# kentril0/WaterSurfaceRendering

Hardware: AMD Instinct MI355X
Metric: ocean frames/s (ComputeWaves, 7 fields -> displacement + normal map) (higher is better)
Workload: dtype f32; 1 GPU; 2048x2048 tile, FULL7, reference default parameters; tile_size=2048, tiles_per_rank=1, pipeline_depth=3, seed=1592590336, parallelism=tiles sharded 1 process per GPU x1, no data-path collective

## Files before the change

watersurfacerendering_amd/csrc/ocean_kernels.h:

```cpp
#pragma once
#include <hip/hip_runtime.h>
#include <hip/hip_fp16.h>
#include <stdint.h>
#include <type_traits>
#include "fft_engine.h"

namespace ocean {

typedef float ocean_f4 __attribute__((ext_vector_type(4)));
__device__ __forceinline__ void store_nt(float4* p, float4 v)
{
    ocean_f4 t = {v.x, v.y, v.z, v.w};
    __builtin_nontemporal_store(t, reinterpret_cast<ocean_f4*>(p));
}
__device__ __forceinline__ void store_f2_sc1(float2* base, unsigned byte_off, float2 v)
{
    typedef float f2v __attribute__((ext_vector_type(2)));
    const f2v t = {v.x, v.y};
    asm volatile("global_store_dwordx2 %0, %1, %2 sc1" ::"v"(byte_off), "v"(t), "s"(base) : "memory");
}
template <bool NTS> __device__ __forceinline__ void store_map(float4* base, unsigned texel, float4 v)
{
    float4* p = reinterpret_cast<float4*>(reinterpret_cast<char*>(base) + (texel * 16u));
    if constexpr (NTS) store_nt(p, v);
// ... 660 lines not shown

template <int N> constexpr size_t zpass_c1_lds_bytes() { return sizeof(c32) * fft_lds_elems<N, 1>() + sizeof(float) * N; }
template <int N, int T, bool FAST> constexpr int zpass_c1_min_waves() { return T == N / 16 ? 3 : (FAST ? 6 : 5); }
template <int N, int T, class P, bool ZNT = false, bool Z16 = false, bool FAST = true, bool ZWT = false>
__global__ void __launch_bounds__(T, (zpass_c1_min_waves<N, T, FAST>())) k_zpass_c1(const FrameArgs a)
{
    extern __shared__ __attribute__((aligned(16))) unsigned char smem[];
    c32* fbuf = reinterpret_cast<c32*>(smem);
    float* sp = reinterpret_cast<float*>(fbuf + fft_lds_elems<N, 1>());
    float* raw = reinterpret_cast<float*>(fbuf);
    const int tid = threadIdx.x;
    const int tile = blockIdx.y;
#ifdef OCEAN_CLOCKPROBE
    ClockProbe clock_probe_(a.frame_seq);
#endif
    start_ramp_wait(a.start_ramp, blockIdx.x, gridDim.x);
    TwiddleRegs<N, 1, T, P> twr;
    twr.load(a.tw, tid);
#ifdef OCEAN_DEVELOPER
    const int bxr = (blockIdx.x % 8 == 0 || a.xcd_rot == 0) ? (int)blockIdx.x : (int)(blockIdx.x / 8 * 8 + 1 + (blockIdx.x % 8 - 1 + a.xcd_rot) % 7);
    const int nb = xcd_swizzle(bxr, N / 2 + 1);
#else
    const int nb = xcd_swizzle((int)blockIdx.x, N / 2 + 1);
#endif
    const float t = a.t + (a.toff ? a.toff[tile] : 0.0f);
    const float* __restrict__ k1 = a.k1d + (size_t)tile * N;
    const bool col0 = (nb == 0);
    const float h16s = a.h0h ? a.h0_inv_scale[tile] : 1.0f;
    const float base = a.omega_q ? a.base_freq[tile] : 0.0f;
    spectrum_form<FAST>(a, [&](auto h16, auto w16) {
        constexpr bool H16 = decltype(h16)::value, W16 = decltype(w16)::value;
        constexpr int PAIRS = N / 2;
        constexpr int P1 = (PAIRS + T - 1) / T;
        constexpr int PB = P1 > 4 ? 4 : P1;
        static_assert(P1 % PB == 0 && PAIRS % T == 0, "phase-1 batches");
#pragma unroll 1
        for (int ub = 0; ub < P1; ub += PB) {
            float4 ha[PB];
            float2 hb0[PB], hb1[PB], wv[PB];
#pragma unroll
            for (int u = 0; u < PB; ++u)
                zpass_load_pair<N, H16, W16, ZNT>(a, tile, nb, 2 * (tid + (ub + u) * T), h16s, base, ha[u], hb0[u], hb1[u], wv[u]);
#pragma unroll
            for (int u = 0; u < PB; ++u) {
                const int n = 2 * (tid + (ub + u) * T);
                float a0, b0, a1, b1;
                animate_with_mirror(make_float2(ha[u].x, ha[u].y), hb0[u], wv[u].x, t, a0, b0);
                animate_with_mirror(make_float2(ha[u].z, ha[u].w), hb1[u], wv[u].y, t, a1, b1);
                *reinterpret_cast<float2*>(sp + n) = col0 ? make_float2(a0, a1) : make_float2(0.5f * (a0 + b0), 0.5f * (a1 + b1));
                if (n == 0) raw[0] = 0.5f * (a0 - b0);
            }
        }
    });
    if (blockIdx.x == 0 && tid == 0 && (a.zmask & 8)) {
        a.minmax[2 * tile + 0] = float_key(3.402823466e+38f);
        a.minmax[2 * tile + 1] = float_key(1.175494351e-38f);
        a.hdone[tile] = 0u;
    }
    float kzr[P::r[0]];
#pragma unroll
    for (int i = 0; i < P::r[0]; ++i) kzr[i] = k1[tid + i * (N / P::r[0])];
    __syncthreads();
    const float sm0 = raw[0];
    static_assert(!ZWT || (!ZNT && !Z16), "write-through is a policy of the plain fp32 intermediates");
    if (col0) zpass_single_transforms<N, T, P, true, ZNT, Z16, ZWT>(a, fbuf, sp, kzr, twr, k1[nb], sm0, tid, tile, nb);
    else zpass_single_transforms<N, T, P, false, ZNT, Z16, ZWT>(a, fbuf, sp, kzr, twr, k1[nb], sm0, tid, tile, nb);
#ifdef OCEAN_CLOCKPROBE
    clock_probe_.end();
#endif
}
template <int N> constexpr bool zpass_has_c1() { return N >= 1024; }
template <int N> inline bool zpass_c1_pays(bool nt_inter, unsigned tiles)
{
    if (N == 4096) return true;
    if (nt_inter) return false;
    return N == 2048 || tiles >= 2;
}

template <int N, int T> constexpr int zpass_blocks_per_cu()
{
    constexpr int by_lds = (int)(163840 / (sizeof(c32) * fft_lds_elems<N, zpass_columns<N>()>() + sizeof(float) * 2 * N));
    constexpr int by_threads = 2048 / T;
    constexpr int by_regs = (zpass_min_waves<N>() * 4 * 64) / T;
    constexpr int m = by_lds < by_threads ? by_lds : by_threads;
    return (by_regs >= 1 && by_regs < m) ? by_regs : (m < 1 ? 1 : m);
}

template <int N, int ZW = 1> constexpr size_t zpass_lds_bytes()
{
    return sizeof(c32) * fft_lds_elems<N, zpass_columns<N>()>() + sizeof(float) * 2 * N;
}


__device__ __forceinline__ void store_wt(float* p, float v) { __hip_atomic_store(p, v, __ATOMIC_RELAXED, __HIP_MEMORY_SCOPE_AGENT); }
__device__ __forceinline__ float load_wt(const float* p) { return __hip_atomic_load(p, __ATOMIC_RELAXED, __HIP_MEMORY_SCOPE_AGENT); }
__device__ __forceinline__ unsigned load_wt(const unsigned* p) { return __hip_atomic_load(p, __ATOMIC_RELAXED, __HIP_MEMORY_SCOPE_AGENT); }
__device__ __forceinline__ void wait_counter(const unsigned* ctr, unsigned target, int tid, int poll_sleep = 0, unsigned* fault = nullptr)
{
    if (tid == 0) {
#ifdef OCEAN_FAULT_INJECT
        target += 1u;
#endif
        const unsigned long long t0 = wall_clock64();
        bool ok;
        while (!(ok = load_wt(ctr) >= target) && (wall_clock64() - t0) < 2000000ull) {
            if (poll_sleep <= 0) __builtin_amdgcn_s_sleep(2);
            else for (int k = 0; k < poll_sleep; ++k) __builtin_amdgcn_s_sleep(127);
        }
        if (!ok && fault) *fault = 1u;
    }
    __syncthreads();
}

__device__ __forceinline__ void wait_counter_reached(const unsigned* ctr, unsigned target, int tid, int poll_sleep = 0, unsigned* fault = nullptr)
{
    if (tid == 0) {
        const unsigned long long t0 = wall_clock64();
        bool ok;
        while (!(ok = (int)(load_wt(ctr) - target) >= 0) && (wall_clock64() - t0) < 2000000ull) {
            if (poll_sleep <= 0) __builtin_amdgcn_s_sleep(2);
            else for (int k = 0; k < poll_sleep; ++k) __builtin_amdgcn_s_sleep(127);
        }
        if (!ok && fault) *fault = 1u;
    }
    __syncthreads();
}

template <int N, bool Z16 = false>
__device__ __forceinline__ c32 load_pair_column(const float2* __restrict__ zg, int mf, int u, float eps, float unscale = 1.0f, float unscale_y = 0.0f)
{
    using HF = Half<N>;
    if (mf <= N / 2) return load_z<Z16>(zg, HF::template zidx<Z16>(mf, 0, u), unscale, unscale_y);
    const int side = (u == 0 || u == N / 2) ? 0 : 1;
    if constexpr (Z16) return load_z<true>(zg, HF::template zidx<Z16>(N - mf, side, u), eps * unscale, eps * unscale_y);
    const c32 v = load_z<false>(zg, HF::template zidx<Z16>(N - mf, side, u), 1.0f);
    return make_float2(eps * v.x, eps * v.y);
}

template <class LS, int T, class F>
__device__ __forceinline__ void for_each_output(int tid, F f)
{
#pragma unroll
    for (int u = 0; u < LS::IT; ++u) {
        const int w = tid + u * T;
        if (!LS::GUARD || w < LS::ITEMS) {
            int c, j;
            LS::map(w, c, j);
#pragma unroll
            for (int i = 0; i < LS::RL; ++i) f(j + i * LS::STRIDE, c, u, i);
        }
    }
}

template <int N, int C> constexpr bool xpass_single_row_group() { return C > 1 && N >= 1024 && (N / 2) % (2 * C) == 0; }
template <int N, int C> constexpr int xpass_height_groups() { return (N / 2 + 1 + 2 * C - 1) / (2 * C); }

constexpr unsigned DONE_GROUPS = 1024, DONE_STRIDE = 16;
template <int T>
__device__ __forceinline__ void frame_done(const FrameArgs& a, unsigned* lds_flag, int tid, unsigned total = 0, unsigned id = 0)
{
    asm volatile("s_waitcnt vmcnt(0)" ::: "memory");
    __syncthreads();
    if (tid == 0) {
        if (total == 0) { total = gridDim.x * gridDim.y; id = blockIdx.y * gridDim.x + blockIdx.x; }
        const unsigned groups = total / 16u < DONE_GROUPS ? (total + 15u) / 16u : DONE_GROUPS;
        const unsigned g = id % groups, members = total / groups + (g < total % groups ? 1u : 0u);
        unsigned* gc = a.done_ctr + (1u + g) * DONE_STRIDE;
        bool last = false;
        if (atomicAdd(gc, 1u) == members - 1u) {
            *gc = 0u;
            last = atomicAdd(a.done_ctr, 1u) == groups - 1u;
        }
        lds_flag[0] = last;
    }
    __syncthreads();
    if (!lds_flag[0]) return;
    if (tid == 0) *a.done_ctr = 0u;
    for (unsigned i = (unsigned)tid; i < gridDim.y; i += (unsigned)T)
        a.done_rec[i] = make_uint4(load_wt(a.minmax + 2 * i + 0), load_wt(a.minmax + 2 * i + 1), a.frame_seq, 0u);
}


template <int T>
__device__ __forceinline__ void frame_records(const FrameArgs& a, unsigned* lds_flag, int tid, bool first_of_tile, unsigned total = 0, unsigned id = 0)
{
    if (a.rec_mode == 1) {
        if (first_of_tile && tid == 0) a.done_rec[blockIdx.y] = make_uint4(load_wt(a.minmax + 2 * blockIdx.y + 0), load_wt(a.minmax + 2 * blockIdx.y + 1), a.frame_seq, 0u);
    } else if (a.rec_mode == 2) {
        frame_done<T>(a, lds_flag, tid, total, id);
    }
}

template <int N, int C, int T, class P, bool NTS, bool Z16, bool JAC, bool ONE = false>
__device__ __forceinline__ void xpass_b_body(const FrameArgs& a, unsigned char* smem, const int bx, const unsigned rec_total = 0, const unsigned rec_id = 0)
{
    using HF = Half<N>;
    c32* fbuf = reinterpret_cast<c32*>(smem);
    const int tid = threadIdx.x;
    const int tile = blockIdx.y;
    constexpr int LM = 1;
    TwiddleRegs<N, C, T, P, LM> twr;
    twr.load(a.tw, tid);
    constexpr int NB = (HF::NU + C - 1) / C;
    constexpr int HB = JAC ? NB : xpass_height_groups<N, C>();
    static_assert(HF::NUP % (2 * C) == 0, "height row blocks");
    if constexpr (ONE) wait_counter_reached(a.zdone + tile, a.zdone_target, tid, a.poll_sleep, a.fault);

    auto pair3_role = [&]() {
    if constexpr (JAC) {
        {
            constexpr int NW = (T + 63) / 64;
            float* red = reinterpret_cast<float*>(fbuf + fft_lds_elems<N, C>());
            const int u0 = xcd_swizzle(bx, HB) * C;
            const float2* __restrict__ z3 = reinterpret_cast<const float2*>(reinterpret_cast<const char*>(a.z3) + (size_t)tile * HF::Z_GROUP * (Z16 ? 4 : 8));
            float* __restrict__ hraw = a.hraw + (size_t)tile * HF::HRAW_TILE;
            float* __restrict__ jraw = a.jraw + (size_t)tile * HF::HRAW_TILE;
            [[maybe_unused]] float ux = 1.0f, uy = 1.0f;
            float ig = 1.0f;
            { const float4 zs3 = a.zscale[2 * tile + 1]; ig = zs3.w; if constexpr (Z16) { ux = zs3.z; uy = zs3.z; } }
            float vmin = 3.402823466e+38f, vmax = -3.402823466e+38f;
            auto in = [&](int nf, int c, int, int) -> c32 { return load_pair_column<N, Z16>(z3, nf, u0 + c, 1.0f, ux, uy); };
            auto out = [&](int p, int c, c32 v, int, int) {
                const int q = u0 + c;
                if (q > N / 2) return;
                const float s = ((p + q) & 1) ? -1.0f : 1.0f;
                const float ha = s * v.x;
                vmin = fminf(vmin, ha); vmax = fmaxf(vmax, ha);
                at32(hraw, hraw_index(N, p, q)) = ha;
                at32(jraw, hraw_index(N, p, q)) = s * v.y * ig;
            };
            batch_fft<N, C, T, P>(fbuf, twr, tid, in, out);
#pragma unroll
            for (int o = 32; o > 0; o >>= 1) {
                vmin = fminf(vmin, __shfl_xor(vmin, o));
                vmax = fmaxf(vmax, __shfl_xor(vmax, o));
            }
            if ((tid & 63) == 0) { red[tid >> 6] = vmin; red[NW + (tid >> 6)] = vmax; }
            __syncthreads();
            if (tid == 0) {
                for (int w = 1; w < NW; ++w) { vmin = fminf(vmin, red[w]); vmax = fmaxf(vmax, red[NW + w]); }
                atomicMin(a.minmax + 2 * tile + 0, float_key(vmin));
                atomicMax(a.minmax + 2 * tile + 1, float_key(vmax));
            }
        }
    }
    };
    auto height_role = [&]() {
        const bool merged = a.xb_disp != 0;
        constexpr int NW = (T + 63) / 64;
        float* red = reinterpret_cast<float*>(fbuf + fft_lds_elems<N, C>());
        const int u0 = xcd_swizzle(bx, HB) * 2 * C;
        constexpr size_t ES = Z16 ? 4 : 8;
        const float2* __restrict__ zh = reinterpret_cast<const float2*>(reinterpret_cast<const char*>(a.zh) + (size_t)tile * HF::ZH_TILE * ES);
        float* __restrict__ hraw = a.hraw + (size_t)tile * HF::HRAW_TILE;
        float vmin = 3.402823466e+38f, vmax = -3.402823466e+38f;
        [[maybe_unused]] const float uu = Z16 ? a.zscale[2 * tile].z : 1.0f;
        auto in = [&](int nf, int c, int, int) -> c32 {
            const int row = nf <= N / 2 ? nf : N - nf;
            float4 z;
            if constexpr (Z16) {
                const float2 raw2 = *reinterpret_cast<const float2*>(reinterpret_cast<const char*>(zh) + HF::template zhidx<Z16>(row, u0 + 2 * c) * 4u);
                __half2 ha, hb;
                __builtin_memcpy(&ha, &raw2.x, 4); __builtin_memcpy(&hb, &raw2.y, 4);
                const float2 fa = __half22float2(ha), fb = __half22float2(hb);
                z = make_float4(fa.x * uu, fa.y * uu, fb.x * uu, fb.y * uu);
            } else {
                z = *reinterpret_cast<const float4*>(&at32(zh, HF::template zhidx<Z16>(row, u0 + 2 * c)));
            }
            if (nf == 0 || nf == N / 2) return make_float2(z.x, z.z);
            if (nf < N / 2) return make_float2(z.x - z.w, z.y + z.z);
            return make_float2(z.x + z.w, z.z - z.y);
        };
        auto out = [&](int p, int c, c32 v, int, int) {
            const int u = u0 + 2 * c;
            const float s = ((p + u) & 1) ? -1.0f : 1.0f;
            const float ha = s * v.x, hb = -s * v.y;
            if (u <= N / 2) { vmin = fminf(vmin, ha); vmax = fmaxf(vmax, ha); }
            if (u + 1 <= N / 2) { vmin = fminf(vmin, hb); vmax = fmaxf(vmax, hb); }
            if (merged) {
                store_wt(&at32(hraw, hraw_index(N, p, u)), ha);
                store_wt(&at32(hraw, hraw_index(N, p, u + 1)), hb);
            } else {
                at32(hraw, hraw_index(N, p, u)) = ha;
                at32(hraw, hraw_index(N, p, u + 1)) = hb;
            }
        };
        if constexpr (xpass_single_row_group<N, C>()) {
            if (u0 == N / 2) {
                TwiddleRegs<N, 1, T, P, LM> tw1;
                tw1.load(a.tw, tid);
                batch_fft<N, 1, T, P>(fbuf, tw1, tid, in, out);
            } else {
                batch_fft<N, C, T, P>(fbuf, twr, tid, in, out);
            }
        } else {
            batch_fft<N, C, T, P>(fbuf, twr, tid, in, out);
        }
#pragma unroll
        for (int o = 32; o > 0; o >>= 1) {
            vmin = fminf(vmin, __shfl_xor(vmin, o));
            vmax = fmaxf(vmax, __shfl_xor(vmax, o));
        }
        if ((tid & 63) == 0) { red[tid >> 6] = vmin; red[NW + (tid >> 6)] = vmax; }
        __syncthreads();
        if (tid == 0) {
            for (int w = 1; w < NW; ++w) { vmin = fminf(vmin, red[w]); vmax = fmaxf(vmax, red[NW + w]); }
            atomicMin(a.minmax + 2 * tile + 0, float_key(vmin));
            atomicMax(a.minmax + 2 * tile + 1, float_key(vmax));
        }
        if (merged) {
            asm volatile("s_waitcnt vmcnt(0)" ::: "memory");
            __syncthreads();
            if (tid == 0) __hip_atomic_fetch_add(a.hdone + tile, 1u, __ATOMIC_RELAXED, __HIP_MEMORY_SCOPE_AGENT);
        }
    };

    using LS = LastStage<N, C, T, P, LM>;
    auto normal_role = [&]() {
    const int nid = bx - HB;
    const int u0 = (N >= 2048 ? (nid == 0 ? NB - 1 : xcd_swizzle(nid - 1, NB - 1)) : xcd_swizzle(nid, NB)) * C;
    start_ramp_wait(a.start_ramp, (unsigned)nid, (unsigned)NB);
    constexpr size_t ESN = Z16 ? 4 : 8;
    const float2* __restrict__ z1 = reinterpret_cast<const float2*>(reinterpret_cast<const char*>(a.z) + ((size_t)tile * HF::Z_TILE + HF::Z_GROUP) * ESN);
    const float2* __restrict__ z2 = reinterpret_cast<const float2*>(reinterpret_cast<const char*>(z1) + HF::Z_GROUP * ESN);
    [[maybe_unused]] const float uk = Z16 ? a.zscale[2 * tile].w : 1.0f;
    float4* __restrict__ nrm = a.nrm + (size_t)tile * N * N;
    float4* __restrict__ nrm_host = a.nrm_host ? a.nrm_host + (size_t)tile * N * N : nullptr;
    [[maybe_unused]] float* __restrict__ jac0 = JAC ? a.jac0 + (size_t)tile * HF::HRAW_TILE : nullptr;
    [[maybe_unused]] const float lambda = a.lambda ? a.lambda[tile] : a.lambda_all;
    c32 held[LS::IT][LS::RL];
    auto emit = [&](int p, int c, c32 slopes, c32 derivs) {
#pragma clang fp contract(off)
        const int q = u0 + c;
        if (q > N / 2) return;
        const float s = ((p + q) & 1) ? -1.0f : 1.0f;
        const float4 o = make_float4(s * slopes.x, s * slopes.y, s * derivs.x, s * derivs.y);
        if constexpr (JAC)
            at32(jac0, hraw_index(N, p, q)) = (1.0f + lambda * o.z) * (1.0f + lambda * o.w);
        OCEAN_STORE(nrm, q * N + p, o);
        store_map_host(nrm_host, (unsigned)(q * N + p), o);
        if (q != 0 && q != N / 2) {
            OCEAN_STORE(nrm, (N - q) * N + ((N - p) & (N - 1)), make_float4(-o.x, -o.y, o.z, o.w));
            store_map_host(nrm_host, (unsigned)((N - q) * N + ((N - p) & (N - 1))), make_float4(-o.x, -o.y, o.z, o.w));
        }
    };
    const c32 zero = make_float2(0.0f, 0.0f);
    if constexpr (xpass_single_row_group<N, C>()) {
        if (u0 == N / 2) {
            using LS1 = LastStage<N, 1, T, P, LM>;
            if (a.mode == 2) {
                for_each_output<LS1, T>(tid, [&](int p, int c, int, int) { emit(p, c, zero, zero); });
                return;
            }
            TwiddleRegs<N, 1, T, P, LM> tw1;
            tw1.load(a.tw, tid);
            c32 held1[LS1::IT][LS1::RL];
            {
                auto in = [&](int nf, int c, int, int) -> c32 { return load_pair_column<N, Z16>(z1, nf, u0 + c, -1.0f, uk); };
                auto out = [&](int, int, c32 v, int u, int i) { held1[u][i] = v; };
                batch_fft<N, 1, T, P>(fbuf, tw1, tid, in, out);
            }
            if (a.mode == 1) {
                for_each_output<LS1, T>(tid, [&](int p, int c, int u, int i) { emit(p, c, held1[u][i], zero); });
                return;
            }
            __builtin_amdgcn_sched_barrier(0);
            auto in = [&](int nf, int c, int, int) -> c32 { return load_pair_column<N, Z16>(z2, nf, u0 + c, 1.0f, uk); };
            auto out = [&](int p, int c, c32 v, int u, int i) { emit(p, c, held1[u][i], v); };
            batch_fft<N, 1, T, P>(fbuf, tw1, tid, in, out);
            return;
        }
    }
    if (a.mode == 2) {
        for_each_output<LS, T>(tid, [&](int p, int c, int, int) { emit(p, c, zero, zero); });
        return;
    }
    constexpr bool PREFETCH = N >= 2048;
    using FS = FirstStage<N, C, T, P>;
    [[maybe_unused]] c32 xb[PREFETCH ? FS::IT : 1][PREFETCH ? FS::R0 : 1];
    auto fetch = [&](const float2* __restrict__ zg, float eps, auto& dst) {
#pragma unroll
        for (int u = 0; u < FS::IT; ++u) {
            const int w = tid + u * T;
            if (!FS::GUARD || w < FS::ITEMS) {
                const int c = w % C, j = w / C;
#pragma unroll
                for (int i = 0; i < FS::R0; ++i) dst[u][i] = load_pair_column<N, Z16>(zg, j + i * FS::STRIDE, u0 + c, eps, uk);
            }
        }
    };
    if constexpr (PREFETCH) {
        c32 xa[FS::IT][FS::R0];
        fetch(z1, -1.0f, xa);
        if (a.mode != 1) fetch(z2, 1.0f, xb);
        auto in = [&](int, int, int u, int i) -> c32 { return xa[u][i]; };
        auto out = [&](int, int, c32 v, int u, int i) { held[u][i] = v; };
        batch_fft<N, C, T, P>(fbuf, twr, tid, in, out);
    } else {
        auto in = [&](int nf, int c, int, int) -> c32 { return load_pair_column<N, Z16>(z1, nf, u0 + c, -1.0f, uk); };
        auto out = [&](int, int, c32 v, int u, int i) { held[u][i] = v; };
        batch_fft<N, C, T, P>(fbuf, twr, tid, in, out);
    }
    if (a.mode == 1) {
        for_each_output<LS, T>(tid, [&](int p, int c, int u, int i) { emit(p, c, held[u][i], zero); });
        return;
    }
    if constexpr (PREFETCH) {
        auto in = [&](int, int, int u, int i) -> c32 { return xb[u][i]; };
        auto out = [&](int p, int c, c32 v, int u, int i) { emit(p, c, held[u][i], v); };
        batch_fft<N, C, T, P>(fbuf, twr, tid, in, out);
    } else {
        __builtin_amdgcn_sched_barrier(0);
        auto in = [&](int nf, int c, int, int) -> c32 { return load_pair_column<N, Z16>(z2, nf, u0 + c, 1.0f, uk); };
        auto out = [&](int p, int c, c32 v, int u, int i) { emit(p, c, held[u][i], v); };
        batch_fft<N, C, T, P>(fbuf, twr, tid, in, out);
    }
    };
    auto disp_role = [&]() {
        if constexpr (!JAC) {
            using LSD = LastStage<N, C, T, P, LM>;
            const int u0 = xcd_swizzle(bx - HB - NB, NB) * C;
            const float2* __restrict__ z0 = reinterpret_cast<const float2*>(reinterpret_cast<const char*>(a.z) + (size_t)tile * HF::Z_TILE * (Z16 ? 4 : 8));
            [[maybe_unused]] const float uu = Z16 ? a.zscale[2 * tile].z : 1.0f;
            const float* __restrict__ hraw = a.hraw + (size_t)tile * HF::HRAW_TILE;
            float4* __restrict__ disp = a.disp + (size_t)tile * N * N;
            float4* __restrict__ disp_host = a.disp_host ? a.disp_host + (size_t)tile * N * N : nullptr;
            c32 dheld[LSD::IT][LSD::RL];
            if (a.mode != 2) {
                auto in = [&](int nf, int c, int, int) -> c32 { return load_pair_column<N, Z16>(z0, nf, u0 + c, -1.0f, uu); };
                auto out = [&](int, int, c32 v, int u, int i) { dheld[u][i] = v; };
                batch_fft<N, C, T, P>(fbuf, twr, tid, in, out);
            } else {
#pragma unroll
                for (int u = 0; u < LSD::IT; ++u)
#pragma unroll
                    for (int i = 0; i < LSD::RL; ++i) dheld[u][i] = make_float2(0.0f, 0.0f);
            }
            wait_counter(a.hdone + tile, (unsigned)HB, tid, a.poll_sleep, a.fault);
            const unsigned kmn = load_wt(a.minmax + 2 * tile + 0), kmx = load_wt(a.minmax + 2 * tile + 1);
            const float mn = key_float(kmn), mx = key_float(kmx);
            const float inv_a = 1.0f / fmaxf(fabsf(mn), fabsf(mx));
            const float lambda = a.lambda ? a.lambda[tile] : a.lambda_all;
            for_each_output<LSD, T>(tid, [&](int p, int c, int u, int i) {
#pragma clang fp contract(off)
                const int q = u0 + c;
                if (q > N / 2) return;
                const float hv = load_wt(&at32(hraw, hraw_index(N, p, q)));
                const float sg = ((p + q) & 1) ? -1.0f : 1.0f;
                const c32 v = dheld[u][i];
                const float4 o = make_float4(sg * lambda * v.x, hv * inv_a, sg * lambda * v.y, 1.0f);
                store_map<NTS>(disp, (unsigned)(q * N + p), o);
                store_map_host(disp_host, (unsigned)(q * N + p), o);
                if (q != 0 && q != N / 2) {
                    store_map<NTS>(disp, (unsigned)((N - q) * N + ((N - p) & (N - 1))), make_float4(-o.x, o.y, -o.z, 1.0f));
                    store_map_host(disp_host, (unsigned)((N - q) * N + ((N - p) & (N - 1))), make_float4(-o.x, o.y, -o.z, 1.0f));
                }
            });
        }
    };
    const bool merged_launch = a.xb_disp != 0;
    if (bx < HB) { if constexpr (JAC) pair3_role(); else height_role(); }
    else if (!JAC && merged_launch && bx >= HB + NB) disp_role();
    else normal_role();
    frame_records<T>(a, reinterpret_cast<unsigned*>(smem), tid, merged_launch ? bx == HB + NB : bx == HB, rec_total, rec_id);
}

template <int N, int C, int T, class P = Plan<N>, bool NTS = false, bool Z16 = false, bool JAC = false>
__global__ void __launch_bounds__(T) k_xpass_b(const FrameArgs a)
{
    extern __shared__ __attribute__((aligned(16))) unsigned char smem[];
    xpass_b_body<N, C, T, P, NTS, Z16, JAC>(a, smem, (int)blockIdx.x);
}

template <int N, int C, int T, class PZ, class PX, bool NTS, bool Z16, bool FAST>
__global__ void __launch_bounds__(T) k_frame(const FrameArgs a)
{
    extern __shared__ __attribute__((aligned(16))) unsigned char smem[];
    using HF = Half<N>;
    constexpr int NZ = N / 2 + 1;
    constexpr int NB = (HF::NU + C - 1) / C, HB = xpass_height_groups<N, C>();
    const int bx = (int)blockIdx.x;
    if (bx < NZ) {
        zpass_body<N, T, PZ, false, Z16, 1, FAST, true>(a, smem, bx, NZ);
        asm volatile("s_waitcnt vmcnt(0)" ::: "memory");
        __syncthreads();
        if (threadIdx.x == 0) __hip_atomic_fetch_add(a.zdone + blockIdx.y, 1u, __ATOMIC_RELAXED, __HIP_MEMORY_SCOPE_AGENT);
        return;
    }
    xpass_b_body<N, C, T, PX, NTS, Z16, false, true>(a, smem, bx - NZ, (unsigned)(HB + 2 * NB) * gridDim.y, (unsigned)blockIdx.y * (unsigned)(HB + 2 * NB) + (unsigned)(bx - NZ));
}

template <int N, int C, int T, class P = Plan<N>, bool NTS = false, bool Z16 = false, bool JAC = false>
__global__ void __launch_bounds__(T, (T == 512 ? 4 : 1)) k_xpass_disp(const FrameArgs a)
{
    extern __shared__ __attribute__((aligned(16))) unsigned char smem[];
    using HF = Half<N>;
    constexpr int LM = 1;
    c32* fbuf = reinterpret_cast<c32*>(smem);
    const int tid = threadIdx.x;
    const int tile = blockIdx.y;
    constexpr int NB = (HF::NU + C - 1) / C;
    const int u0 = xcd_swizzle(blockIdx.x, NB) * C;
    start_ramp_wait(a.start_ramp, blockIdx.x, gridDim.x);
    const float2* __restrict__ z0 = reinterpret_cast<const float2*>(reinterpret_cast<const char*>(a.z) + (size_t)tile * HF::Z_TILE * (Z16 ? 4 : 8));
    [[maybe_unused]] const float uu = Z16 ? a.zscale[2 * tile].z : 1.0f;
    const float* __restrict__ hraw = a.hraw + (size_t)tile * HF::HRAW_TILE;
    float4* __restrict__ disp = a.disp + (size_t)tile * N * N;
    float4* __restrict__ disp_host = a.disp_host ? a.disp_host + (size_t)tile * N * N : nullptr;
    auto rows = [&](auto cc_tag) {
        constexpr int CC = decltype(cc_tag)::value;
        using LS = LastStage<N, CC, T, P, LM>;
        TwiddleRegs<N, CC, T, P, LM> twr;
        twr.load(a.tw, tid);
        float hv[LS::IT][LS::RL];
        [[maybe_unused]] float jv[JAC ? LS::IT : 1][JAC ? LS::RL : 1], j0[JAC ? LS::IT : 1][JAC ? LS::RL : 1];
#pragma unroll
        for (int u = 0; u < LS::IT; ++u) {
            const int w = tid + u * T;
            if (!LS::GUARD || w < LS::ITEMS) {
                int c, j;
                LS::map(w, c, j);
#pragma unroll
                for (int i = 0; i < LS::RL; ++i) {
                    hv[u][i] = at32(hraw, hraw_index(N, j + i * LS::STRIDE, u0 + c));
                    if constexpr (JAC) {
                        jv[u][i] = at32(a.jraw + (size_t)tile * HF::HRAW_TILE, hraw_index(N, j + i * LS::STRIDE, u0 + c));
                        j0[u][i] = at32(a.jac0 + (size_t)tile * HF::HRAW_TILE, hraw_index(N, j + i * LS::STRIDE, u0 + c));
                    }
                }
            }
        }
        const unsigned kmn = a.minmax[2 * tile + 0], kmx = a.minmax[2 * tile + 1];
        if (a.rec_mode == 1 && blockIdx.x == 0 && tid == 0) a.done_rec[tile] = make_uint4(kmn, kmx, a.frame_seq, 0u);
        const float mn = key_float(kmn);
        const float mx = key_float(kmx);
        const float inv_a = 1.0f / fmaxf(fabsf(mn), fabsf(mx));
        const float lambda = a.lambda ? a.lambda[tile] : a.lambda_all;
        auto in = [&](int nf, int c, int, int) -> c32 { return load_pair_column<N, Z16>(z0, nf, u0 + c, -1.0f, uu); };
        auto out = [&](int p, int c, c32 v, int u, int i) {
#pragma clang fp contract(off)
            const int q = u0 + c;
            if (q > N / 2) return;
            const float s = ((p + q) & 1) ? -1.0f : 1.0f;
            float w = 1.0f;
            if constexpr (JAC) {
                const float cross = lambda * jv[u][i];
                w = j0[u][i] - cross * cross;
            }
            const float4 o = make_float4(s * lambda * v.x, hv[u][i] * inv_a, s * lambda * v.y, w);
            OCEAN_STORE(disp, q * N + p, o);
            store_map_host(disp_host, (unsigned)(q * N + p), o);
            if (q != 0 && q != N / 2) {
                OCEAN_STORE(disp, (N - q) * N + ((N - p) & (N - 1)), make_float4(-o.x, o.y, -o.z, w));
                store_map_host(disp_host, (unsigned)((N - q) * N + ((N - p) & (N - 1))), make_float4(-o.x, o.y, -o.z, w));
            }
        };
        if (a.mode == 2)
            for_each_output<LS, T>(tid, [&](int p, int c, int u, int i) { out(p, c, make_float2(0.0f, 0.0f), u, i); });
        else
            batch_fft<N, CC, T, P>(fbuf, twr, tid, in, out);
    };
    if constexpr (xpass_single_row_group<N, C>()) {
        if (u0 == N / 2) rows(std::integral_constant<int, 1>{});
        else rows(std::integral_constant<int, C>{});
    } else {
        rows(std::integral_constant<int, C>{});
    }
    if (a.rec_mode == 2) frame_done<T>(a, reinterpret_cast<unsigned*>(smem), tid);
}


template <int N> struct Geo;
#define OCEAN_R(...) Radices<__VA_ARGS__>
#define OCEAN_GEO(n, tr, pr, cc, tc, pc)                                                       \
    template <> struct Geo<n> {                                                                \
        static constexpr int T_ROWS = tr;                \
        static constexpr int CC = cc, T_C = tc;          \
        using PR = pr; using PC = pc;                    \
    };
OCEAN_GEO(16, 64, Plan<16>, 4, 64, Plan<16>)
OCEAN_GEO(32, 64, Plan<32>, 4, 64, Plan<32>)
OCEAN_GEO(64, 64, Plan<64>, 4, 64, Plan<64>)
OCEAN_GEO(128, 64, Plan<128>, 4, 64, Plan<128>)
OCEAN_GEO(256, 64, Plan<256>, 4, 64, Plan<256>)
OCEAN_GEO(512, (zpass_columns<512>() == 4 ? 256 : 128), Plan<512>, 4, 256, Plan<512>)
OCEAN_GEO(1024, 256, OCEAN_R(8, 8, 4, 4), 4, 256, Plan<1024>)
OCEAN_GEO(2048, 512, OCEAN_R(8, 8, 8, 4), 4, 512, Plan<2048>)
OCEAN_GEO(4096, 1024, OCEAN_R(8, 8, 8, 8), 2, 512, Plan<4096>)
#undef OCEAN_GEO

template <int N> constexpr bool zpass_c1_r16() { return N >= 8192; }
template <int N> constexpr int zpass_c1_threads() { return zpass_c1_r16<N>() ? N / 16 : N / 8; }
template <int N> struct C1Plan { using type = std::conditional_t<zpass_c1_r16<N>(), Plan<N>, typename Geo<N>::PR>; };

}
```

watersurfacerendering_amd/csrc/ocean_launch.h:

```cpp
#pragma once
#include <cstdlib>

#include "ocean_ctx.h"

using namespace ocean;

template <class K>
static hipError_t allow_lds(K kernel, size_t bytes)
{
    if (bytes <= 48 * 1024) return hipSuccess;
    return hipFuncSetAttribute(reinterpret_cast<const void*>(kernel), hipFuncAttributeMaxDynamicSharedMemorySize,
                               (int)bytes);
}

template <class K, class... A>
static void launch(K kernel, dim3 grid, dim3 block, size_t lds, hipStream_t st, hipEvent_t* ev, A... args)
{
    if (ev) hipExtLaunchKernelGGL(kernel, grid, block, (uint32_t)lds, st, ev[0], ev[1], 0, args...);
    else hipLaunchKernelGGL(kernel, grid, block, lds, st, args...);
}

template <int N> constexpr bool xmerge_pays(bool alone) { return alone ? N <= 128 : N <= 512; }

template <int N>
static hipError_t launch_frame(ocean_ctx* c, const FrameArgs& a, FrameLaunch& fl)
{
    const FramePolicy& p = fl.policy;
    const hipStream_t st = fl.stream;
    using G = Geo<N>;
    using HF = Half<N>;
    const unsigned tiles = c->tiles;
    hipError_t e;
    constexpr int C = G::CC;
    constexpr size_t lds_rows = zpass_lds_bytes<N, 1>();
    constexpr bool HAS2 = zpass_has_width2<N>();
    constexpr size_t lds_rows2 = zpass_lds_bytes<N, 2>();
    constexpr size_t lds_m = sizeof(c32) * fft_lds_elems<N, C>();
    constexpr size_t lds_b = lds_m + sizeof(float) * 2 * ((G::T_C + 63) / 64);
    static_assert(HF::NUP % (2 * C) == 0, "height row blocks");
    constexpr unsigned hb_b = xpass_height_groups<N, C>(), nb = (HF::NU + C - 1) / C;
    const bool fast = !a.h0h && a.omega_q;
    const bool alone = p.alone;
    const unsigned cus = (unsigned)(c->cu_count > 0 ? c->cu_count : 0);
    int ramp_z = 0, ramp_b = 0, ramp_d = 0;
#ifdef OCEAN_DEVELOPER
    constexpr bool DEV = true;
#else
    constexpr bool DEV = false;
#endif
    constexpr bool HAS1 = DEV || N <= 1024;
    constexpr bool HASC1 = zpass_has_c1<N>();
    constexpr bool HAS2_PLAIN = DEV && HAS2;
    if (c->attr_n != (uint32_t)N) {
#define OCEAN_ALLOW_Z(znt, z16, fast) \
        if constexpr (HAS1) if ((e = allow_lds(k_zpass<N, G::T_ROWS, typename G::PR, znt, z16, 1, fast>, lds_rows)) != hipSuccess) return e; \
        if constexpr (HAS2 && (znt || HAS2_PLAIN)) if ((e = allow_lds(k_zpass<N, G::T_ROWS, typename G::PR, znt, z16, 2, fast>, lds_rows2)) != hipSuccess) return e; \
        if constexpr (HASC1) if ((e = allow_lds(k_zpass_c1<N, zpass_c1_threads<N>(), typename C1Plan<N>::type, znt, z16, fast>, zpass_c1_lds_bytes<N>())) != hipSuccess) return e; \
        if constexpr (HASC1 && zpass_has_wt<N>() && !znt && !z16) if ((e = allow_lds(k_zpass_c1<N, zpass_c1_threads<N>(), typename C1Plan<N>::type, false, false, fast, true>, zpass_c1_lds_bytes<N>())) != hipSuccess) return e;
#define OCEAN_ALLOW_Z2(fast) OCEAN_ALLOW_Z(false, false, fast) OCEAN_ALLOW_Z(true, false, fast) OCEAN_ALLOW_Z(false, true, fast) OCEAN_ALLOW_Z(true, true, fast)
        OCEAN_ALLOW_Z2(true) OCEAN_ALLOW_Z2(false)
#undef OCEAN_ALLOW_Z2
#undef OCEAN_ALLOW_Z
#define OCEAN_ALLOW_X1(kern, lds, z16, jac) \
        if ((e = allow_lds(kern<N, C, G::T_C, typename G::PC, false, z16, jac>, lds)) != hipSuccess) return e; \
        if ((e = allow_lds(kern<N, C, G::T_C, typename G::PC, true, z16, jac>, lds)) != hipSuccess) return e;
#define OCEAN_ALLOW_X2(kern, lds, jac) OCEAN_ALLOW_X1(kern, lds, false, jac) OCEAN_ALLOW_X1(kern, lds, true, jac)
#define OCEAN_ALLOW_X(kern, lds) OCEAN_ALLOW_X2(kern, lds, false) OCEAN_ALLOW_X2(kern, lds, true)
        OCEAN_ALLOW_X(k_xpass_b, lds_b)
        OCEAN_ALLOW_X(k_xpass_disp, lds_m)
#undef OCEAN_ALLOW_X
#undef OCEAN_ALLOW_X2
#undef OCEAN_ALLOW_X1
        c->attr_n = (uint32_t)N;
    }
    if (c->start_ramp && cus) {
        if (c->occ_n != N) {
            int oz = 0, oza = 0, ob = 0, od = 0;
            if constexpr (zpass_has_c1<N>()) {
                (void)hipOccupancyMaxActiveBlocksPerMultiprocessor(&oz, k_zpass_c1<N, zpass_c1_threads<N>(), typename C1Plan<N>::type, false, false, true>,
                                                                   zpass_c1_threads<N>(), zpass_c1_lds_bytes<N>());
                (void)hipOccupancyMaxActiveBlocksPerMultiprocessor(&oza, k_zpass_c1<N, zpass_c1_threads<N>(), typename C1Plan<N>::type, false, false, false>,
                                                                   zpass_c1_threads<N>(), zpass_c1_lds_bytes<N>());
            }
            (void)hipOccupancyMaxActiveBlocksPerMultiprocessor(&ob, k_xpass_b<N, C, G::T_C, typename G::PC, false, false, false>, G::T_C, lds_b);
            (void)hipOccupancyMaxActiveBlocksPerMultiprocessor(&od, k_xpass_disp<N, C, G::T_C, typename G::PC, false, false, false>, G::T_C, lds_m);
            (void)hipGetLastError();
            c->occ_z = oz; c->occ_z_all = oza; c->occ_b = ob; c->occ_d = od; c->occ_n = N;
        }
        int bpt[3];
        ocean_launch_bytes_per_texel(p.half_inter, a.mode == 3, a.h0h != nullptr, a.omega_q != nullptr, bpt);
        const OceanTuning& tu = c->tune;
        const double texels = (double)tiles * N * N;
        auto ramp_ticks = [&](int bytes_per_texel, unsigned workgroups, int per_cu, double scale) -> int {
            const double bytes = texels * bytes_per_texel;
            const unsigned slots = (unsigned)per_cu < tu.ramp_max_wg_per_cu ? (unsigned)per_cu : tu.ramp_max_wg_per_cu;
            if (per_cu <= 0 || workgroups > slots * cus || texels < tu.ramp_min_texels) return 0;
            return (int)(tu.ramp_frac * scale * bytes / tu.ramp_rate_bytes_per_s * 1.0e8 + 0.5);
        };
        ramp_z = ramp_ticks(bpt[0], (unsigned)(N / 2 + 1) * tiles, fast ? c->occ_z : c->occ_z_all, 1.0);
        ramp_b = ramp_ticks(bpt[1] - 4, (hb_b + nb) * tiles, c->occ_b, alone ? 1.0 : tu.ramp_pipelined_x);
        ramp_d = ramp_ticks(bpt[2], nb * tiles, c->occ_d, alone ? 1.0 : tu.ramp_pipelined_x);
    }
    bool c1 = HASC1 && zpass_c1_pays<N>(p.nt_inter, tiles);
    bool zw2 = HAS2 && !c1 && p.nt_inter;
    constexpr bool HAS_WT = HASC1 && zpass_has_wt<N>();
    const bool wt_frame = HAS_WT && alone && !p.nt_inter && !p.half_inter && c->z_write_through;
    bool z_wt = c1 && wt_frame;
    bool merged_x = xmerge_pays<N>(alone) && tiles == 1 && a.mode != 3 && c->merged_x &&
                    (hb_b + 2u * nb) <= c->tune.handoff_wg_per_cu * cus;
    constexpr bool HAS_ONE = (N <= 128 || (DEV && N <= 512)) && G::T_ROWS == G::T_C;
    bool one_launch = HAS_ONE && !alone && tiles == 1 && a.mode <= 2 && fast && p.nt_normal && p.nt_disp && !p.nt_inter && !p.half_inter && c->merged_x &&
                      ((unsigned)(N / 2 + 1) + hb_b + 2u * nb) <= c->tune.handoff_wg_per_cu * cus;
    int poll_sleep = (merged_x && !one_launch && !alone) ? 1 : 0;
#ifdef OCEAN_DEVELOPER
    {   static const char* const c1_env = getenv("OCEAN_ZC1");
        if (c1_env && HASC1) c1 = atoi(c1_env) != 0;
        zw2 = HAS2 && !c1 && p.nt_inter;
        static const char* const zw_env = getenv("OCEAN_ZW");
        if (zw_env && HAS2 && !c1) zw2 = atoi(zw_env) == 2;
        const char* const wt_env = getenv("OCEAN_Z_WT");
        z_wt = c1 && wt_frame && !(wt_env && atoi(wt_env) == 0);
        const char* const xm = getenv("OCEAN_XMERGE");
        if (xm) merged_x = atoi(xm) != 0 && a.mode != 3;
        const char* const ol = getenv("OCEAN_ONE_LAUNCH");
        if (ol) one_launch = one_launch && atoi(ol) != 0;
        const char* const ps = getenv("OCEAN_POLL_SLEEP");
        poll_sleep = ps ? atoi(ps) : (merged_x && !one_launch && !alone) ? 1 : 0;
        static const char* const rz = getenv("OCEAN_RAMP_Z"); static const char* const rb = getenv("OCEAN_RAMP_B"); static const char* const rd = getenv("OCEAN_RAMP_D");
        static const char* const ra = getenv("OCEAN_RAMP_ANY");
        const bool on = ramp_z || ramp_b || ramp_d || (ra && atoi(ra) == 1);
        if (rz && on) ramp_z = atoi(rz);
        if (rb && on) ramp_b = atoi(rb);
        if (rd && on) ramp_d = atoi(rd); }
#endif
    fl.handoff = merged_x || one_launch;
    fl.launch_count = 0;
    auto next_marks = [&](int kernel) -> hipEvent_t* {
        const int l = fl.launch_count++;
        fl.launch_kernel[l] = kernel;
        return fl.marks ? fl.marks + 2 * l : nullptr;
    };
    auto describe = [&](int idx, unsigned grid_x, unsigned block, unsigned per_workgroup, size_t lds, uint32_t flags) {
        ocean_launch_info& li = c->last_launch[idx];
        li.tile_size = N; li.grid_x = grid_x; li.grid_y = tiles; li.block = block; li.mode = (uint32_t)a.mode;
        li.per_workgroup = per_workgroup;
        li.lds_bytes = (uint32_t)lds;
        li.flags = flags | (p.half_inter ? OCEAN_LAUNCH_HALF_INTER : 0u) | (a.mode == 3 ? OCEAN_LAUNCH_JACOBIAN : 0u);
    };
    const int rec_last = a.rec_mode;
    auto launch_z = [&]() -> hipError_t {
        const unsigned gx = zw2 ? N / 4 + 1 : N / 2 + 1;
        FrameArgs za = a;
        za.rec_mode = 0;
        za.start_ramp = c1 ? ramp_z : 0;
        const unsigned threads = c1 ? (unsigned)zpass_c1_threads<N>() : (unsigned)G::T_ROWS;
        const size_t lds = c1 ? zpass_c1_lds_bytes<N>() : (zw2 ? lds_rows2 : lds_rows);
        const dim3 grid(gx, tiles), block(threads);
        describe(0, gx, threads, zw2 ? 2u : 1u, lds,
                 (p.nt_inter ? OCEAN_LAUNCH_NT_INTER : 0u) | (a.h0h ? OCEAN_LAUNCH_FP16_SPECTRUM : 0u) |
                 (a.omega_q ? 0u : OCEAN_LAUNCH_FP32_DISPERSION) | (c1 ? OCEAN_LAUNCH_SINGLE_TRANSFORM : 0u) |
                 (za.start_ramp ? OCEAN_LAUNCH_STAGGERED_START : 0u) | (z_wt ? OCEAN_LAUNCH_WT_INTER : 0u));
        hipEvent_t* mz = next_marks(0);
#ifdef OCEAN_CLOCKPROBE
        {
            static unsigned long long* armed = nullptr;
            if (armed != c->stamps) { armed = c->stamps; (void)hipMemcpyToSymbol(HIP_SYMBOL(ocean::g_clockprobe), &armed, sizeof(armed)); }
        }
#endif
        bool launched = false;
        if constexpr (HAS_WT) {
            if (z_wt) {
                if (fast) launch(k_zpass_c1<N, zpass_c1_threads<N>(), typename C1Plan<N>::type, false, false, true, true>, grid, block, lds, st, mz, za);
                else launch(k_zpass_c1<N, zpass_c1_threads<N>(), typename C1Plan<N>::type, false, false, false, true>, grid, block, lds, st, mz, za);
                launched = true;
            }
        }
#define OCEAN_ZPASS3(znt, z16, fast) \
        do { if (launched) break; if constexpr (HASC1) { if (c1) { launch(k_zpass_c1<N, zpass_c1_threads<N>(), typename C1Plan<N>::type, znt, z16, fast>, grid, block, lds, st, mz, za); launched = true; break; } } \
             if constexpr (HAS2 && (znt || HAS2_PLAIN)) { if (zw2) { launch(k_zpass<N, G::T_ROWS, typename G::PR, znt, z16, 2, fast>, grid, block, lds, st, mz, za); launched = true; break; } } \
             if constexpr (HAS1) { if (!c1 && !zw2) { launch(k_zpass<N, G::T_ROWS, typename G::PR, znt, z16, 1, fast>, grid, block, lds, st, mz, za); launched = true; } } } while (0)
#define OCEAN_ZPASS2(znt, z16) \
        do { if (fast) OCEAN_ZPASS3(znt, z16, true); else OCEAN_ZPASS3(znt, z16, false); } while (0)
#define OCEAN_ZPASS(znt) \
        do { if (p.half_inter) OCEAN_ZPASS2(znt, true); else OCEAN_ZPASS2(znt, false); } while (0)
        if (p.nt_inter) OCEAN_ZPASS(true); else OCEAN_ZPASS(false);
#undef OCEAN_ZPASS
#undef OCEAN_ZPASS2
#undef OCEAN_ZPASS3
        if (!launched) return hipErrorInvalidConfiguration;
        return hipSuccess;
    };
// ... 67 lines not shown
```

Baseline: 21540 frames/s.

## Rotate mirrored texel stores across lanes so conjugate writes stay contiguous

The x-pass output now writes the Hermitian-mirrored half of the normal and displacement maps with each lane storing its neighbour's value, fetched via a DPP lane shift. Wave-boundary values are handed off through a small LDS buffer. This makes the mirrored stores ascend in address order within a wave instead of descending, so they coalesce better. In exchange it holds both FFT results in registers until the end, adds a barrier and LDS space, and asserts the LDS budget still allows two workgroups per CU.

```diff
diff --git a/watersurfacerendering_amd/csrc/ocean_kernels.h b/watersurfacerendering_amd/csrc/ocean_kernels.h
--- a/watersurfacerendering_amd/csrc/ocean_kernels.h
+++ b/watersurfacerendering_amd/csrc/ocean_kernels.h
@@ -836,6 +836,51 @@
     }
 }
 
+template <int N, int C, int T, class P, int LM, bool NTS = true> constexpr bool mirror_rotates()
+{
+    return NTS && LM == 1 && C > 1 && (N / P::last) % 64 == 0 && T % 64 == 0 && ((N / P::last) * C) % T == 0;
+}
+template <int N, int C, int T, class P> constexpr size_t mirror_handoff_bytes() { return mirror_rotates<N, C, T, P, 1>() ? sizeof(float4) * C * (N / 64) : 0; }
+template <int N, int C, int T> constexpr size_t mirror_handoff_offset() { return (sizeof(c32) * fft_lds_elems<N, C>() + sizeof(float) * 2 * ((T + 63) / 64) + 15) / 16 * 16; }
+__device__ __forceinline__ float wave_next_lane(float v)
+{
+    return __builtin_bit_cast(float, __builtin_amdgcn_update_dpp(0, __builtin_bit_cast(int, v), 0x134, 0xf, 0xf, false));
+}
+template <int N, class LS, int T, class V>
+__device__ __forceinline__ void publish_row_heads(float4* hand, int tid, int u0, V value)
+{
+    for_each_output<LS, T>(tid, [&](int p, int c, int u, int i) {
+        if ((tid & 63) == 0) hand[c * (N / 64) + (p >> 6)] = value(p, u0 + c, u, i);
+    });
+}
+template <int N, class LS, int T, bool NTS, class V, class S, class M>
+__device__ __forceinline__ void store_rows_whole(float4* __restrict__ map, float4* __restrict__ map_host, const float4* hand, int tid, int u0, V value, S side, M mirror)
+{
+    __syncthreads();
+    for_each_output<LS, T>(tid, [&](int p, int c, int u, int i) {
+        const int q = u0 + c;
+        const float4 o = value(p, q, u, i);
+        float4 nx = make_float4(wave_next_lane(o.x), wave_next_lane(o.y), wave_next_lane(o.z), wave_next_lane(o.w));
+        if ((tid & 63) == 63) nx = hand[c * (N / 64) + (((p >> 6) + 1) & (N / 64 - 1))];
+        if (q > N / 2) return;
+        side(p, q, o);
+        store_map<NTS>(map, (unsigned)(q * N + p), o);
+        store_map_host(map_host, (unsigned)(q * N + p), o);
+        if (q == 0 || q == N / 2) return;
+        const unsigned t = (unsigned)((N - q) * N + (N - 1 - p));
+        const float4 m = mirror(nx);
+        store_map<NTS>(map, t, m);
+        store_map_host(map_host, t, m);
+    });
+}
+template <int A, int B> __device__ __forceinline__ void launder(c32 (&x)[A][B])
+{
+#pragma unroll
+    for (int u = 0; u < A; ++u)
+#pragma unroll
+        for (int i = 0; i < B; ++i) asm volatile("" : "+v"(x[u][i].x), "+v"(x[u][i].y));
+}
+
 template <int N, int C> constexpr bool xpass_single_row_group() { return C > 1 && N >= 1024 && (N / 2) % (2 * C) == 0; }
 template <int N, int C> constexpr int xpass_height_groups() { return (N / 2 + 1 + 2 * C - 1) / (2 * C); }
 
@@ -1013,14 +1058,21 @@
     [[maybe_unused]] float* __restrict__ jac0 = JAC ? a.jac0 + (size_t)tile * HF::HRAW_TILE : nullptr;
     [[maybe_unused]] const float lambda = a.lambda ? a.lambda[tile] : a.lambda_all;
     c32 held[LS::IT][LS::RL];
+    auto texel = [&](int p, int q, c32 slopes, c32 derivs) -> float4 {
+#pragma clang fp contract(off)
+        const float s = ((p + q) & 1) ? -1.0f : 1.0f;
+        return make_float4(s * slopes.x, s * slopes.y, s * derivs.x, s * derivs.y);
+    };
+    auto jac_factor = [&]([[maybe_unused]] int p, [[maybe_unused]] int q, [[maybe_unused]] float4 o) {
+#pragma clang fp contract(off)
+        if constexpr (JAC)
+            at32(jac0, hraw_index(N, p, q)) = (1.0f + lambda * o.z) * (1.0f + lambda * o.w);
+    };
     auto emit = [&](int p, int c, c32 slopes, c32 derivs) {
-#pragma clang fp contract(off)
         const int q = u0 + c;
         if (q > N / 2) return;
-        const float s = ((p + q) & 1) ? -1.0f : 1.0f;
-        const float4 o = make_float4(s * slopes.x, s * slopes.y, s * derivs.x, s * derivs.y);
-        if constexpr (JAC)
-            at32(jac0, hraw_index(N, p, q)) = (1.0f + lambda * o.z) * (1.0f + lambda * o.w);
+        const float4 o = texel(p, q, slopes, derivs);
+        jac_factor(p, q, o);
         OCEAN_STORE(nrm, q * N + p, o);
         store_map_host(nrm_host, (unsigned)(q * N + p), o);
         if (q != 0 && q != N / 2) {
@@ -1029,6 +1081,24 @@
         }
     };
     const c32 zero = make_float2(0.0f, 0.0f);
+    constexpr bool ROT = mirror_rotates<N, C, T, P, LM, NTS>();
+    [[maybe_unused]] c32 held2[ROT ? LS::IT : 1][ROT ? LS::RL : 1];
+    [[maybe_unused]] auto fill = [&](auto& x, c32 v) {
+#pragma unroll
+        for (int u = 0; u < LS::IT; ++u)
+#pragma unroll
+            for (int i = 0; i < LS::RL; ++i) x[u][i] = v;
+    };
+    [[maybe_unused]] auto store_rows = [&]() {
+        if constexpr (ROT) {
+            float4* hand = reinterpret_cast<float4*>(smem + mirror_handoff_offset<N, C, T>());
+            auto value = [&](int p, int q, int u, int i) { return texel(p, q, held[u][i], held2[u][i]); };
+            publish_row_heads<N, LS, T>(hand, tid, u0, value);
+            launder(held);
+            launder(held2);
+            store_rows_whole<N, LS, T, NTS>(nrm, nrm_host, hand, tid, u0, value, jac_factor, [](float4 o) { return make_float4(-o.x, -o.y, o.z, o.w); });
+        }
+    };
     if constexpr (xpass_single_row_group<N, C>()) {
         if (u0 == N / 2) {
             using LS1 = LastStage<N, 1, T, P, LM>;
@@ -1056,7 +1126,8 @@
         }
     }
     if (a.mode == 2) {
-        for_each_output<LS, T>(tid, [&](int p, int c, int, int) { emit(p, c, zero, zero); });
+        if constexpr (ROT) { fill(held, zero); fill(held2, zero); store_rows(); }
+        else for_each_output<LS, T>(tid, [&](int p, int c, int, int) { emit(p, c, zero, zero); });
         return;
     }
     constexpr bool PREFETCH = N >= 2048;
@@ -1086,19 +1157,23 @@
         batch_fft<N, C, T, P>(fbuf, twr, tid, in, out);
     }
     if (a.mode == 1) {
-        for_each_output<LS, T>(tid, [&](int p, int c, int u, int i) { emit(p, c, held[u][i], zero); });
+        if constexpr (ROT) { fill(held2, zero); store_rows(); }
+        else for_each_output<LS, T>(tid, [&](int p, int c, int u, int i) { emit(p, c, held[u][i], zero); });
         return;
     }
+    auto out = [&](int p, int c, c32 v, int u, int i) {
+        if constexpr (ROT) held2[u][i] = v;
+        else emit(p, c, held[u][i], v);
+    };
     if constexpr (PREFETCH) {
         auto in = [&](int, int, int u, int i) -> c32 { return xb[u][i]; };
-        auto out = [&](int p, int c, c32 v, int u, int i) { emit(p, c, held[u][i], v); };
         batch_fft<N, C, T, P>(fbuf, twr, tid, in, out);
     } else {
         __builtin_amdgcn_sched_barrier(0);
         auto in = [&](int nf, int c, int, int) -> c32 { return load_pair_column<N, Z16>(z2, nf, u0 + c, 1.0f, uk); };
-        auto out = [&](int p, int c, c32 v, int u, int i) { emit(p, c, held[u][i], v); };
         batch_fft<N, C, T, P>(fbuf, twr, tid, in, out);
     }
+    store_rows();
     };
     auto disp_role = [&]() {
         if constexpr (!JAC) {
@@ -1221,17 +1296,21 @@
         const float inv_a = 1.0f / fmaxf(fabsf(mn), fabsf(mx));
         const float lambda = a.lambda ? a.lambda[tile] : a.lambda_all;
         auto in = [&](int nf, int c, int, int) -> c32 { return load_pair_column<N, Z16>(z0, nf, u0 + c, -1.0f, uu); };
-        auto out = [&](int p, int c, c32 v, int u, int i) {
+        auto texel = [&](int p, int q, c32 v, int u, int i) -> float4 {
 #pragma clang fp contract(off)
-            const int q = u0 + c;
-            if (q > N / 2) return;
             const float s = ((p + q) & 1) ? -1.0f : 1.0f;
             float w = 1.0f;
             if constexpr (JAC) {
                 const float cross = lambda * jv[u][i];
                 w = j0[u][i] - cross * cross;
             }
-            const float4 o = make_float4(s * lambda * v.x, hv[u][i] * inv_a, s * lambda * v.y, w);
+            return make_float4(s * lambda * v.x, hv[u][i] * inv_a, s * lambda * v.y, w);
+        };
+        auto out = [&](int p, int c, c32 v, int u, int i) {
+            const int q = u0 + c;
+            if (q > N / 2) return;
+            const float4 o = texel(p, q, v, u, i);
+            const float w = o.w;
             OCEAN_STORE(disp, q * N + p, o);
             store_map_host(disp_host, (unsigned)(q * N + p), o);
             if (q != 0 && q != N / 2) {
@@ -1239,7 +1318,19 @@
                 store_map_host(disp_host, (unsigned)((N - q) * N + ((N - p) & (N - 1))), make_float4(-o.x, o.y, -o.z, w));
             }
         };
-        if (a.mode == 2)
+        if constexpr (mirror_rotates<N, CC, T, P, LM, NTS>()) {
+            c32 vh[LS::IT][LS::RL];
+            auto hold = [&](int, int, c32 v, int u, int i) { vh[u][i] = v; };
+            if (a.mode == 2)
+                for_each_output<LS, T>(tid, [&](int p, int c, int u, int i) { hold(p, c, make_float2(0.0f, 0.0f), u, i); });
+            else
+                batch_fft<N, CC, T, P>(fbuf, twr, tid, in, hold);
+            float4* hand = reinterpret_cast<float4*>(smem + mirror_handoff_offset<N, C, T>());
+            auto value = [&](int p, int q, int u, int i) { return texel(p, q, vh[u][i], u, i); };
+            publish_row_heads<N, LS, T>(hand, tid, u0, value);
+            launder(vh);
+            store_rows_whole<N, LS, T, NTS>(disp, disp_host, hand, tid, u0, value, [](int, int, float4) {}, [](float4 o) { return make_float4(-o.x, o.y, -o.z, o.w); });
+        } else if (a.mode == 2)
             for_each_output<LS, T>(tid, [&](int p, int c, int u, int i) { out(p, c, make_float2(0.0f, 0.0f), u, i); });
         else
             batch_fft<N, CC, T, P>(fbuf, twr, tid, in, out);
diff --git a/watersurfacerendering_amd/csrc/ocean_launch.h b/watersurfacerendering_amd/csrc/ocean_launch.h
--- a/watersurfacerendering_amd/csrc/ocean_launch.h
+++ b/watersurfacerendering_amd/csrc/ocean_launch.h
@@ -35,8 +35,10 @@
     constexpr size_t lds_rows = zpass_lds_bytes<N, 1>();
     constexpr bool HAS2 = zpass_has_width2<N>();
     constexpr size_t lds_rows2 = zpass_lds_bytes<N, 2>();
-    constexpr size_t lds_m = sizeof(c32) * fft_lds_elems<N, C>();
-    constexpr size_t lds_b = lds_m + sizeof(float) * 2 * ((G::T_C + 63) / 64);
+    constexpr size_t lds_hand = mirror_handoff_bytes<N, C, G::T_C, typename G::PC>();
+    constexpr size_t lds_m = lds_hand ? mirror_handoff_offset<N, C, G::T_C>() + lds_hand : sizeof(c32) * fft_lds_elems<N, C>();
+    constexpr size_t lds_b = lds_hand ? lds_m : sizeof(c32) * fft_lds_elems<N, C>() + sizeof(float) * 2 * ((G::T_C + 63) / 64);
+    static_assert(lds_b <= 80 * 1024, "two x-pass workgroups per compute unit");
     static_assert(HF::NUP % (2 * C) == 0, "height row blocks");
     constexpr unsigned hb_b = xpass_height_groups<N, C>(), nb = (HF::NU + C - 1) / C;
     const bool fast = !a.h0h && a.omega_q;
```

Measured after the change: 22230 frames/s, median of 6. +3.2%, better.
